# MECLabTUDA/Lifelong-nnUNet

Hardware: AMD Instinct MI355X
Metric: 3D patches/sec (whole node) + mean Dice vs ref, 5-level 3D Generic_UNet training step (higher is better)
Workload: dtype f16 (fp32 accumulate, fp32 master weights); 1 GPU; BASELINE configs[1]: nnUNetTrainerSequential.run_iteration, 160x192x160 patches, batch 2/GPU, num_pool 5, base 32, 3 logits; global_batch=2, parallelism=dp1, distinct_resident_batches=2, deterministic_wgrad=False

## Files before the change

lifelong-nnunet_amd/csrc/igemm_wgrad.hip:

```cpp
#include "lnn_common.h"
#include "igemm_gen.h"
#include <cstdlib>

namespace {

struct WTapTable {
    int ntaps;
    unsigned short pos_off[27];
    unsigned char slot[27];
};

struct WgradParams {
    const half_t* p;
    const half_t* q;
    const half_t* q2 = nullptr;
    int csplit = 0x7fffffff;
    float* dwp;
    int ld_p, ld_q;
    int N, Ld, Lh, Lw, Qd, Qh, Qw;
    int M, C, Mpad, Cpad;
    int tiles_z, tiles_y, tiles_x, tiles_total, tiles_per_block;
    int pad_lo;
    float* parts = nullptr;
    long parts_elems = 0, part_stride = 0;
// ... 748 lines not shown
                const char* qa = smem + 2 * ch * QX * 64 + tapaddr[ti];
                bq[buf][0] = lds_tr16(qa);
                bq[buf][1] = lds_tr16(qa + 256);
            }
        };
        rdA(0, 0);
        rdB(0, 0);
#pragma unroll
        for (int g = 0; g < NG; ++g) {
            const int ch = g / TPW, ti = g % TPW;
            if (g + 1 < NG) {
                rdB(g + 1, (g + 1) & 1);
                if ((g + 1) % TPW == 0) rdA((g + 1) / TPW, ((g + 1) / TPW) & 1);
            }
            if (wave + 8 * ti < NTAP) {
                const half4 b0 = bq[g & 1][0], b1 = bq[g & 1][1];
                const half8 b = {b0[0], b0[1], b0[2], b0[3], b1[0], b1[1], b1[2], b1[3]};
#pragma unroll
                for (int mp = 0; mp < MP; ++mp) acc[ti][mp] = __builtin_amdgcn_mfma_f32_32x32x16_f16(a[ch & 1][mp], b, acc[ti][mp], 0, 0, 0);
            }
#pragma unroll
            for (int e = 0; e < DPP; ++e) {
                const int d = g * DPP + e;
                if (d < nq) dma_q(nxt, rel0 + d / KPW, wrap(nbase + rel0 + d / KPW), d % KPW);
                else if (d == nq) dma_p(nxt, img ^ 1);
            }
            __builtin_amdgcn_sched_barrier(0);
        }
        wg_wait_all();
        __syncthreads();
        base = nbase;
        img ^= 1;
        cur = nxt;
    }
    const int c = c0 + (lane & 31);
#pragma unroll
    for (int ti = 0; ti < TPW; ++ti) {
        const int tap = wave + 8 * ti;
        if (tap < NTAP) {
            const long pbase_ = (long)tap * p.Mpad * p.Cpad;
#pragma unroll
            for (int mp = 0; mp < MP; ++mp) {
                if (m0 + mp * 32 >= p.Mpad) continue;
#pragma unroll
                for (int r = 0; r < 16; ++r) {
                    const int m = m0 + mp * 32 + 8 * (r >> 2) + 4 * hk + (r & 3);
                    wg_out(p, blk.chunk, 0, pbase_ + (long)m * p.Cpad + c, acc[ti][mp][r]);
                }
            }
        }
    }
}

int launch_wgrad_s1_v5(hipStream_t s, WgradParams& p) {
    constexpr int TZ = 4, TY = 8, TX = 8;
    p.tiles_z = lnn_cdiv(p.Ld, TZ); p.tiles_y = lnn_cdiv(p.Lh, TY); p.tiles_x = lnn_cdiv(p.Lw, TX);
    p.tiles_total = p.N * p.tiles_z * p.tiles_y * p.tiles_x;
    const int panels = (p.Mpad / 32) * (p.Cpad / 32);
    static int num_cu = 0;
    if (!num_cu) {
        int dev = 0;
        hipDeviceProp_t prop;
        num_cu = (hipGetDevice(&dev) == hipSuccess && hipGetDeviceProperties(&prop, dev) == hipSuccess) ? prop.multiProcessorCount : 256;
        hipFuncSetAttribute(reinterpret_cast<const void*>(igemm_wgrad_s1_v5_kernel), hipFuncAttributeMaxDynamicSharedMemorySize, 160 * 1024);
    }
    static int dbg4 = -1;
    static unsigned long long* dbgbuf4 = nullptr;
    if (dbg4 < 0) {
        const char* e = getenv("LNN_WGRAD_DEBUG"); dbg4 = e ? atoi(e) : 0;
        const char* b = getenv("LNN_WGRAD_PHASEBUF"); if ((dbg4 & 4) && b) dbgbuf4 = (unsigned long long*)strtoull(b, nullptr, 0);
    }
    p.debug = dbg4; p.dbgbuf = dbgbuf4;
    int tpb = lnn_cdiv((long)p.tiles_total * panels, lnn_cu_budget(num_cu));
    if (tpb < 1) tpb = 1;
    if (tpb > p.tiles_total) tpb = p.tiles_total;
    p.tiles_per_block = tpb;
    const unsigned chunks = (unsigned)lnn_cdiv(p.tiles_total, tpb);
    const dim3 grid = wg_grid(p, chunks, (unsigned)panels);
    const long slot_elems = 27L * p.Mpad * p.Cpad;
    if (int e = wg_prepare_parts(p, chunks, 2, slot_elems, "lnn_conv3d_wgrad(s1)")) return e;
    hipLaunchKernelGGL(igemm_wgrad_s1_v5_kernel, grid, dim3(512), (size_t)(12 * 7 * 1024 + 2 * 2 * 512 * 16), s, p);
    LNN_CHECK_LAUNCH("lnn_conv3d_wgrad(s1,v5)");
    return wg_reduce_parts(s, p, chunks, slot_elems, "lnn_conv3d_wgrad(s1,v5,reduce)");
}

template <int EXT>
int launch_wgrad_s2_v2(hipStream_t s, WgradParams& p, const char* name) {
    constexpr int TY = 8, TX = 8;
    constexpr int QZ = 1 + (EXT == 3), QY = TY + (EXT == 3), QX = TX + (EXT == 3);
    p.tiles_z = p.Ld; p.tiles_y = lnn_cdiv(p.Lh, TY); p.tiles_x = lnn_cdiv(p.Lw, TX);
    p.tiles_total = p.N * p.tiles_z * p.tiles_y * p.tiles_x;
    const int panels = lnn_cdiv(p.Mpad, 64) * (p.Cpad / 32);
    int tpb = lnn_cdiv((long)p.tiles_total * panels, 512);
    if (tpb < 1) tpb = 1;
    if (tpb > p.tiles_total) tpb = p.tiles_total;
    p.tiles_per_block = tpb;
    const size_t lds = (size_t)8 * QZ * QY * QX * 64 + (size_t)2 * 64 * 64;
    auto kern = igemm_wgrad_s2_v2_kernel<EXT>;
    static bool attr_set = false;
    if (!attr_set) {
        (void)hipFuncSetAttribute(reinterpret_cast<const void*>(kern), hipFuncAttributeMaxDynamicSharedMemorySize, 159 * 1024);
        attr_set = true;
    }
    const unsigned chunks = (unsigned)lnn_cdiv(p.tiles_total, tpb);
    const dim3 grid = wg_grid(p, chunks, (unsigned)panels);
    const long slot_elems = (long)(EXT * EXT * EXT) * p.Mpad * p.Cpad;
    if (int e = wg_prepare_parts(p, chunks, 1, slot_elems, name)) return e;
    hipLaunchKernelGGL(kern, grid, dim3(512), lds, s, p);
    LNN_CHECK_LAUNCH(name);
    return wg_reduce_parts(s, p, chunks, slot_elems, name);
}

template <int EXT>
int launch_wgrad_s2(hipStream_t s, WgradParams& p, const char* name) {
    static int s2s = -1;
    if (s2s < 0) { const char* e = getenv("LNN_WGRAD_S2S"); s2s = (e && e[0] == '0') ? 0 : 1; }
    constexpr int TY = 8, TX = 8, PY = 2 * (TY - 1) + EXT;
    const bool dma_ok = (long)PY * p.Qw * p.ld_q * 2 < 0x7fffffffL && (long)TY * p.Lw * p.ld_p * 2 < 0x7fffffffL;
    const bool one_panel_ext2 = EXT == 2 && lnn_cdiv(p.Mpad, 64) * (p.Cpad / 32) < 2;
    if (!s2s || !dma_ok || one_panel_ext2) return launch_wgrad_s2_v2<EXT>(s, p, name);
    constexpr int QY = TY + (EXT == 3), QX = TX + (EXT == 3), NPI = (4 * QY * QX * 64 + 1023) / 1024;
    p.tiles_z = p.Ld; p.tiles_y = lnn_cdiv(p.Lh, TY); p.tiles_x = lnn_cdiv(p.Lw, TX);
    p.tiles_total = p.N * p.tiles_z * p.tiles_y * p.tiles_x;
    const int panels = lnn_cdiv(p.Mpad, 64) * (p.Cpad / 32);
    static int num_cu = 0;
    if (!num_cu) {
        int dev = 0;
        hipDeviceProp_t prop;
        num_cu = (hipGetDevice(&dev) == hipSuccess && hipGetDeviceProperties(&prop, dev) == hipSuccess) ? prop.multiProcessorCount : 256;
    }
    int tpb = lnn_cdiv((long)p.tiles_total * panels, lnn_cu_budget(num_cu));
    if (tpb < 1) tpb = 1;
    if (tpb > p.tiles_total) tpb = p.tiles_total;
    p.tiles_per_block = tpb;
    const size_t lds = (size_t)2 * EXT * NPI * 1024 + (size_t)2 * 2 * 64 * 64;
    auto kern = igemm_wgrad_s2s_kernel<EXT>;
    static bool attr_set = false;
    if (!attr_set) {
        (void)hipFuncSetAttribute(reinterpret_cast<const void*>(kern), hipFuncAttributeMaxDynamicSharedMemorySize, 160 * 1024);
        attr_set = true;
    }
    const unsigned chunks = (unsigned)lnn_cdiv(p.tiles_total, tpb);
    const dim3 grid = wg_grid(p, chunks, (unsigned)panels);
    const long slot_elems = (long)(EXT * EXT * EXT) * p.Mpad * p.Cpad;
    if (int e = wg_prepare_parts(p, chunks, 1, slot_elems, name)) return e;
    hipLaunchKernelGGL(kern, grid, dim3(512), lds, s, p);
    LNN_CHECK_LAUNCH(name);
    return wg_reduce_parts(s, p, chunks, slot_elems, name);
}

int check_act_w(const void* ptr, int ld, int C, const char* what) {
    LNN_REQUIRE(ptr != nullptr, "%s: null pointer", what);
    LNN_REQUIRE(lnn_aligned16(ptr), "%s: pointer not 16-byte aligned", what);
    LNN_REQUIRE(C > 0 && C % 8 == 0, "%s: channel count %d must be a positive multiple of 8", what, C);
    LNN_REQUIRE(ld >= C && ld % 8 == 0, "%s: ld %d must be >= C (%d) and a multiple of 8", what, ld, C);
    return LNN_OK;
}

}

namespace {
__global__ void tr16_probe_kernel(float* out) {
    __shared__ __attribute__((aligned(16))) half_t img[256];
    for (int i = threadIdx.x; i < 256; i += 64) img[i] = (half_t)(float)i;
    __syncthreads();
    const half4 r = lds_tr16(reinterpret_cast<const char*>(img) + threadIdx.x * 8);
    for (int j = 0; j < 4; ++j) out[threadIdx.x * 4 + j] = (float)r[j];
}
}

extern "C" int lnn_debug_tr16_probe(lnn_stream_t s_, float* out256) {
    LNN_REQUIRE(out256 != nullptr, "lnn_debug_tr16_probe: null pointer");
    hipLaunchKernelGGL(tr16_probe_kernel, dim3(1), dim3(64), 0, (hipStream_t)s_, out256);
    LNN_CHECK_LAUNCH("lnn_debug_tr16_probe");
    return LNN_OK;
}

extern "C" size_t lnn_wgrad_panel_elems(int ntaps, int M, int KC) {
    return (size_t)ntaps * lnn_round_up(M, 32) * lnn_round_up(KC, 32);
}

namespace {
struct C1Fused {
    const void* gz; int ld_gz; const float *mean, *rstd, *gamma, *beta; float slope; const double* sums;
};
int conv3d_wgrad_impl(lnn_stream_t s_, const void* x, const void* x2, int c_a, int ld_x, const void* dy, int ld_dy, float* dwp, int N,
                      int Di, int Hi, int Wi, int C, int K, int stride, float* parts = nullptr, long parts_elems = 0,
                      const C1Fused* fused = nullptr) {
    hipStream_t s = (hipStream_t)s_;
    LNN_REQUIRE(stride == 1 || stride == 2, "lnn_conv3d_wgrad: stride %d unsupported", stride);
    LNN_REQUIRE(dwp != nullptr, "lnn_conv3d_wgrad: null panel");
    if (int e = check_act_w(dy, ld_dy, K, "lnn_conv3d_wgrad(dy)")) return e;
    WgradParams p{};
    p.p = (const half_t*)dy; p.q = (const half_t*)x; p.dwp = dwp; p.ld_p = ld_dy; p.ld_q = ld_x;
    p.parts = parts; p.parts_elems = parts_elems;
    if (x2) { p.q2 = (const half_t*)x2; p.csplit = c_a; }
    p.N = N; p.Qd = Di; p.Qh = Hi; p.Qw = Wi;
    p.Ld = (Di - 1) / stride + 1; p.Lh = (Hi - 1) / stride + 1; p.Lw = (Wi - 1) / stride + 1;
    p.M = K; p.C = C; p.Mpad = lnn_round_up(K, 32); p.Cpad = lnn_round_up(C, 32); p.pad_lo = 1;
    if (fused) {
        LNN_REQUIRE(C == 1, "lnn_conv3d_wgrad_c1_in_bwd: first layer (C == 1) only");
        p.gz = (const half_t*)fused->gz; p.ld_gz = fused->ld_gz; p.in_mean = fused->mean; p.in_rstd = fused->rstd;
        p.in_gamma = fused->gamma; p.in_beta = fused->beta; p.in_slope = fused->slope; p.in_sums = fused->sums;
    }
    if (C == 1) {
        LNN_REQUIRE(stride == 1 && x != nullptr, "lnn_conv3d_wgrad: C == 1 path needs stride 1");
        constexpr int TZ = 4, TY = 8;
        p.Cpad = 32;
        p.tiles_z = lnn_cdiv(p.Ld, TZ); p.tiles_y = lnn_cdiv(p.Lh, TY); p.tiles_x = lnn_cdiv(p.Lw, 8);
        p.tiles_total = N * p.tiles_z * p.tiles_y * p.tiles_x;
        int tpb = lnn_cdiv(p.tiles_total, 2048);
        if (tpb < 1) tpb = 1;
        p.tiles_per_block = tpb;
        dim3 grid((unsigned)lnn_cdiv(p.tiles_total, tpb), (unsigned)(p.Mpad / 32));
        const long slot_elems = (long)p.Mpad * 32;
        if (int e = wg_prepare_parts(p, grid.x, 4, slot_elems, "lnn_conv3d_wgrad(C=1)")) return e;
        if (p.gz) hipLaunchKernelGGL((wgrad_c1_kernel<TZ, TY, true>), grid, dim3(256), 0, s, p);
        else hipLaunchKernelGGL((wgrad_c1_kernel<TZ, TY, false>), grid, dim3(256), 0, s, p);
        LNN_CHECK_LAUNCH("lnn_conv3d_wgrad(C=1)");
        return wg_reduce_parts(s, p, grid.x, slot_elems, "lnn_conv3d_wgrad(C=1,reduce)");
    }
    if (int e = check_act_w(x, ld_x, x2 ? c_a : C, "lnn_conv3d_wgrad(x)")) return e;
    if (!x2 && lnn_gen_prefers(LNN_GEN_OP_WGRAD, (long)N * p.Ld * p.Lh * p.Lw)) {
        const int k3[3] = {3, 3, 3}, st3[3] = {stride, stride, stride};
        return lnn_gen_conv3d_wgrad(s, x, ld_x, dy, ld_dy, dwp, N, Di, Hi, Wi, C, K, k3, st3, parts, parts_elems);
    }
    p.taps.ntaps = 27;
    if (stride == 1) {
        constexpr int PY = 10, PX = 10;
        for (int t = 0; t < 27; ++t) {
            p.taps.pos_off[t] = (unsigned short)(((t / 9) * PY + (t / 3) % 3) * PX + t % 3);
            p.taps.slot[t] = (unsigned char)t;
        }
        LNN_REQUIRE(6L * p.Qh * p.Qw * p.ld_q * 2 < 0x7fffffffL && 4L * p.Lh * p.Lw * p.ld_p * 2 < 0x7fffffffL,
                    "lnn_conv3d_wgrad: a z-plane of %ld bytes is beyond the 2 GB window of the tile descriptors", (long)p.Qh * p.Qw * p.ld_q * 2);
        return launch_wgrad_s1_v5(s, p);
    }
    return launch_wgrad_s2<3>(s, p, "lnn_conv3d_wgrad(s2)");
}
}

extern "C" int lnn_conv3d_wgrad(lnn_stream_t s, const void* x, int ld_x, const void* dy, int ld_dy, float* dwp, int N,
                                int Di, int Hi, int Wi, int C, int K, int stride) {
    return conv3d_wgrad_impl(s, x, nullptr, 0, ld_x, dy, ld_dy, dwp, N, Di, Hi, Wi, C, K, stride);
}

extern "C" int lnn_conv3d_wgrad_c1_in_bwd(lnn_stream_t s, const void* x, const void* y, const void* dz, int ld_dz, float* dwp, int N,
                                          int D, int H, int W, int K, const float* mean, const float* rstd, const float* gamma,
                                          const float* beta, float slope, const double* ws, float* parts, long parts_elems) {
    LNN_REQUIRE(y && dz && lnn_aligned16(y) && lnn_aligned16(dz) && ld_dz >= K && ld_dz % 8 == 0, "lnn_conv3d_wgrad_c1_in_bwd: bad y / dz / ld_dz");
    LNN_REQUIRE(mean && rstd && gamma && beta && ws, "lnn_conv3d_wgrad_c1_in_bwd: null parameter");
    LNN_REQUIRE(parts == nullptr || lnn_aligned16(parts), "lnn_conv3d_wgrad_c1_in_bwd: scratch misaligned");
    const C1Fused f{dz, ld_dz, mean, rstd, gamma, beta, slope, ws};
    return conv3d_wgrad_impl(s, x, nullptr, 0, 1, y, K, dwp, N, D, H, W, 1, K, 1, parts, parts_elems, &f);
}

extern "C" int lnn_conv3d_wgrad_cat(lnn_stream_t s, const void* x_a, const void* x_b, int ld_x, int c_a, const void* dy, int ld_dy,
                                    float* dwp, int N, int Di, int Hi, int Wi, int C, int K) {
    LNN_REQUIRE(x_b != nullptr && lnn_aligned16(x_b), "lnn_conv3d_wgrad_cat: second tensor null/misaligned");
    LNN_REQUIRE(c_a > 0 && c_a < C && c_a % 32 == 0 && (C - c_a) % 8 == 0, "lnn_conv3d_wgrad_cat: split %d of %d channels must be a multiple of 32", c_a, C);
    LNN_REQUIRE(ld_x >= c_a && ld_x >= C - c_a, "lnn_conv3d_wgrad_cat: ld_x %d smaller than a part (%d / %d)", ld_x, c_a, C - c_a);
    return conv3d_wgrad_impl(s, x_a, x_b, c_a, ld_x, dy, ld_dy, dwp, N, Di, Hi, Wi, C, K, 1);
}

namespace {
int convT3d_k2s2_wgrad_impl(lnn_stream_t s_, const void* x, int ld_x, const void* dy, int ld_dy, float* dwp, int N, int D, int H, int W,
                            int C, int K, float* parts, long parts_elems);
}
extern "C" int lnn_convT3d_k2s2_wgrad(lnn_stream_t s, const void* x, int ld_x, const void* dy, int ld_dy, float* dwp,
                                      int N, int D, int H, int W, int C, int K) {
    return convT3d_k2s2_wgrad_impl(s, x, ld_x, dy, ld_dy, dwp, N, D, H, W, C, K, nullptr, 0);
}
extern "C" int lnn_conv3d_wgrad_det(lnn_stream_t s, const void* x, int ld_x, const void* dy, int ld_dy, float* dwp, int N, int Di, int Hi,
                                    int Wi, int C, int K, int stride, float* parts, long parts_elems) {
    LNN_REQUIRE(parts != nullptr && lnn_aligned16(parts), "lnn_conv3d_wgrad_det: scratch null/misaligned");
    return conv3d_wgrad_impl(s, x, nullptr, 0, ld_x, dy, ld_dy, dwp, N, Di, Hi, Wi, C, K, stride, parts, parts_elems);
}
extern "C" int lnn_conv3d_wgrad_cat_det(lnn_stream_t s, const void* x_a, const void* x_b, int ld_x, int c_a, const void* dy, int ld_dy,
                                        float* dwp, int N, int Di, int Hi, int Wi, int C, int K, float* parts, long parts_elems) {
    LNN_REQUIRE(parts != nullptr && lnn_aligned16(parts), "lnn_conv3d_wgrad_cat_det: scratch null/misaligned");
    LNN_REQUIRE(x_b != nullptr && lnn_aligned16(x_b), "lnn_conv3d_wgrad_cat_det: second tensor null/misaligned");
    LNN_REQUIRE(c_a > 0 && c_a < C && c_a % 32 == 0 && (C - c_a) % 8 == 0, "lnn_conv3d_wgrad_cat_det: split %d of %d channels must be a multiple of 32", c_a, C);
    LNN_REQUIRE(ld_x >= c_a && ld_x >= C - c_a, "lnn_conv3d_wgrad_cat_det: ld_x %d smaller than a part (%d / %d)", ld_x, c_a, C - c_a);
    return conv3d_wgrad_impl(s, x_a, x_b, c_a, ld_x, dy, ld_dy, dwp, N, Di, Hi, Wi, C, K, 1, parts, parts_elems);
}
extern "C" int lnn_convT3d_k2s2_wgrad_det(lnn_stream_t s, const void* x, int ld_x, const void* dy, int ld_dy, float* dwp, int N, int D,
                                          int H, int W, int C, int K, float* parts, long parts_elems) {
    LNN_REQUIRE(parts != nullptr && lnn_aligned16(parts), "lnn_convT3d_k2s2_wgrad_det: scratch null/misaligned");
    return convT3d_k2s2_wgrad_impl(s, x, ld_x, dy, ld_dy, dwp, N, D, H, W, C, K, parts, parts_elems);
}
namespace {
int convT3d_k2s2_wgrad_impl(lnn_stream_t s_, const void* x, int ld_x, const void* dy, int ld_dy, float* dwp, int N, int D, int H, int W,
                            int C, int K, float* parts, long parts_elems) {
    hipStream_t s = (hipStream_t)s_;
    LNN_REQUIRE(dwp != nullptr, "lnn_convT3d_k2s2_wgrad: null panel");
    if (int e = check_act_w(x, ld_x, C, "lnn_convT3d_k2s2_wgrad(x)")) return e;
    if (int e = check_act_w(dy, ld_dy, K, "lnn_convT3d_k2s2_wgrad(dy)")) return e;
    if (lnn_gen_prefers(LNN_GEN_OP_WGRAD, (long)N * D * H * W)) {
        const int st3[3] = {2, 2, 2};
        return lnn_gen_convT3d_wgrad(s, x, ld_x, dy, ld_dy, dwp, N, D, H, W, C, K, st3, parts, parts_elems);
    }
    WgradParams p{};
    p.p = (const half_t*)x; p.q = (const half_t*)dy; p.dwp = dwp; p.ld_p = ld_x; p.ld_q = ld_dy;
    p.parts = parts; p.parts_elems = parts_elems;
    p.N = N; p.Ld = D; p.Lh = H; p.Lw = W; p.Qd = 2 * D; p.Qh = 2 * H; p.Qw = 2 * W;
    p.M = C; p.C = K; p.Mpad = lnn_round_up(C, 32); p.Cpad = lnn_round_up(K, 32); p.pad_lo = 0;
    return launch_wgrad_s2<2>(s, p, "lnn_convT3d_k2s2_wgrad");
}
}
```

lifelong-nnunet_amd/csrc/lnn_debug.h:

```cpp
#ifndef LNN_DEBUG_H
#define LNN_DEBUG_H
#include "../../include/lnn_hip.h"
#ifdef __cplusplus
extern "C" {
#endif

int lnn_debug_tr16_probe(lnn_stream_t s, float* out256);

int lnn_debug_set_phase_buffer(void* dev_ptr_6x_u64);
int lnn_debug_force_conv_kernel(int which);
int lnn_debug_force_down2_kernel(int which);
int lnn_debug_set_v9_zseg(int segments);

int lnn_debug_set_k133_v9(int mode);
int lnn_debug_last_k133_on_v9(void);

int lnn_debug_set_gen_mode(int mode);

int lnn_debug_last_dgrad_reduce_fused(void);

int lnn_debug_set_cu_budget(int cus);

#ifdef __cplusplus
}
#endif
#endif
```

lifelong-nnunet_amd/native.py:

```python
from __future__ import annotations

import ctypes as C
import os

_HERE = os.path.dirname(os.path.abspath(__file__))
LIB_PATH = os.environ.get("LNN_LIB_PATH") or os.path.join(_HERE, "csrc", "liblnn_hip.so")

_p = C.c_void_p
_i = C.c_int
_l = C.c_long
_f = C.c_float
_sz = C.c_size_t

SIGNATURES = {
    "lnn_last_error": (C.c_char_p, []),
    "lnn_version": (_i, []),
    "lnn_device_info": (_i, [C.POINTER(_i), C.POINTER(_i), C.c_char_p, _i]),
    "lnn_pack_weights": (_i, [_p, _p, _p, _i, _i, _i, _l, _l, _l]),
    "lnn_packed_weight_elems": (_sz, [_i, _i, _i]),
    "lnn_conv3d_fwd": (_i, [_p, _p, _i, _p, _p, _p, _i, _i, _i, _i, _i, _i, _i, _i]),
    "lnn_conv3d_dgrad": (_i, [_p, _p, _i, _p, _p, _i, _i, _i, _i, _i, _i, _i, _i, _i]),
    "lnn_conv3d_wgrad": (_i, [_p, _p, _i, _p, _i, _p, _i, _i, _i, _i, _i, _i, _i]),
    "lnn_conv3d_fwd_cat": (_i, [_p, _p, _p, _i, _i, _p, _p, _p, _i, _i, _i, _i, _i, _i, _i]),
    "lnn_conv3d_fwd_in_stats": (_i, [_p, _p, _p, _i, _i, _p, _p, _p, _i, _i, _i, _i, _i, _i, _i, _f, _p, _p, _p, _p, _l]),
# ... 30 lines not shown
    "lnn_seg1x1_bwd_ws_floats": (_sz, [_i, _i]),
    "lnn_dice_ce_fwd": (_i, [_p, _p, _p, _i, _i, _l, _i, _f, _p, _p]),
    "lnn_dice_ce_fwd_ds": (_i, [_p, _p, _p, _i, _i, _l, _i, _f, _p, _p, _f, _p, _i]),
    "lnn_dice_ce_bwd": (_i, [_p, _p, _p, _i, _i, _l, _i, _f, _p, _f, _p, _f, _p]),
    "lnn_dice_ce_loss_from_totals": (_i, [_p, _p, _i, _i, _l, _i, _f, _p]),
    "lnn_dice_ce_ws_doubles": (_sz, [_i, _i]),
    "lnn_online_dice_counts": (_i, [_p, _p, _p, _i, _i, _l, _p]),
    "lnn_kl_logits": (_i, [_p, _p, _p, _i, _i, _l, _f, _p, _p]),
    "lnn_kl_logits_ws_doubles": (_sz, [_i]),
    "lnn_plop_pseudo_labels": (_i, [_p, _p, _p, _p, _f, _i, _i, _i, _i, _i, _p, _p, _p, _p]),
    "lnn_local_pod": (_i, [_p, _p, _p, _i, _i, _i, _i, _i, _l, _l, _l, _l, _l, _i, _f, _i, _p, _p, _p]),
    "lnn_ewc_penalty_fwd": (_i, [_p, _p, _p, _p, _l, _f, _p, _p]),
    "lnn_ewc_penalty_bwd": (_i, [_p, _p, _p, _p, _l, _f, _f, _p, _p]),
    "lnn_fisher_square": (_i, [_p, _p, _p, _l, _f]),
    "lnn_fisher_accumulate": (_i, [_p, _p, _p, _l, _f, _f]),
    "lnn_fisher_ema": (_i, [_p, _p, _p, _l, _f, _f]),
    "lnn_rw_update": (_i, [_p, _p, _p, _p, _p, _p, _l, _f, _f, _p, _f, _f, _i]),
    "lnn_target_ce_fwd": (_i, [_p, _p, _p, _i, _i, _i, _l, _f, _i, _f, _p, _p]),
    "lnn_target_ce_bwd": (_i, [_p, _p, _p, _i, _i, _i, _l, _f, _i, _f, _p, _f, _p, _p]),
    "lnn_softmax_accumulate": (_i, [_p, _p, _p, _p, _p] + [_i] * 11 + [_f, _i]),
    "lnn_softmax_finalize": (_i, [_p, _p, _p, _i, _l, _p]),
    "lnn_gradnorm_sumsq": (_i, [_p, _p, _l, _f, _p, _i]),
    "lnn_flat_reduce_ws_doubles": (_sz, []),
    "lnn_sgd_nesterov_step_clipped": (_i, [_p, _p, _p, _p, _l, _f, _f, _f, _f, _f, _p]),
    "lnn_sgd_nesterov_step": (_i, [_p, _p, _p, _p, _l, _f, _f, _f, _f, _i]),
    "lnn_cast_f32_to_h": (_i, [_p, _p, _p, _l]),
    "lnn_f32_conv3d_fwd": (_i, [_p, _p, _i, _p, _p, _p, _i, _i, _i, _i, _i, _i, _i, _i]),
    "lnn_f32_conv3d_dgrad": (_i, [_p, _p, _i, _p, _p, _i, _i, _i, _i, _i, _i, _i, _i, _i]),
    "lnn_f32_conv3d_wgrad": (_i, [_p, _p, _i, _p, _i, _p, _i, _i, _i, _i, _i, _i, _i]),
    "lnn_f32_convT3d_k2s2_fwd": (_i, [_p, _p, _i, _p, _p, _i, _i, _i, _i, _i, _i, _i]),
    "lnn_f32_convT3d_k2s2_dgrad": (_i, [_p, _p, _i, _p, _p, _i, _i, _i, _i, _i, _i, _i, _i]),
    "lnn_f32_convT3d_k2s2_wgrad": (_i, [_p, _p, _i, _p, _i, _p, _i, _i, _i, _i, _i, _i]),
    "lnn_f32_conv3d_fwd_g": (_i, [_p, _p, _i, _p, _p, _p, _i] + [_i] * 12),
    "lnn_f32_conv3d_dgrad_g": (_i, [_p, _p, _i, _p, _p, _i] + [_i] * 13),
    "lnn_f32_conv3d_wgrad_g": (_i, [_p, _p, _i, _p, _i, _p] + [_i] * 12),
    "lnn_f32_convT3d_fwd_g": (_i, [_p, _p, _i, _p, _p, _i] + [_i] * 9),
    "lnn_f32_convT3d_dgrad_g": (_i, [_p, _p, _i, _p, _p, _i] + [_i] * 10),
    "lnn_f32_convT3d_wgrad_g": (_i, [_p, _p, _i, _p, _i, _p] + [_i] * 9),
    "lnn_image_to_cl_h": (_i, [_p, _p, _p, _i, _i, _l, _i]),
    "lnn_f32_image_to_cl": (_i, [_p, _p, _p, _i, _i, _l, _i]),
    "lnn_f32_instnorm_lrelu_fwd": (_i, [_p, _p, _i, _p, _i, _i, _l, _i, _f, _p, _p, _p, _p, _f]),
    "lnn_f32_instnorm_lrelu_bwd": (_i, [_p, _p, _i, _p, _i, _i, _l, _i, _p, _p, _p, _p, _f, _p, _p, _p]),
    "lnn_f32_seg1x1_fwd": (_i, [_p, _p, _i, _p, _p, _i, _l, _i, _i]),
    "lnn_f32_seg1x1_bwd": (_i, [_p, _p, _i, _p, _p, _p, _i, _p, _i, _l, _i, _i, _i]),
    "lnn_debug_tr16_probe": (_i, [_p, _p]),
    "lnn_debug_set_phase_buffer": (_i, [_p]),
    "lnn_debug_force_conv_kernel": (_i, [_i]),
    "lnn_debug_force_down2_kernel": (_i, [_i]),
    "lnn_debug_set_v9_zseg": (_i, [_i]),
    "lnn_debug_set_k133_v9": (_i, [_i]),
    "lnn_debug_last_k133_on_v9": (_i, []),
    "lnn_debug_set_gen_mode": (_i, [_i]),
    "lnn_debug_last_dgrad_reduce_fused": (_i, []),
    "lnn_debug_set_cu_budget": (_i, [_i]),
    "lnn_conv3d_fwd_g": (_i, [_p, _p, _i, _p, _p, _p, _i] + [_i] * 12 + [_p, _l]),
    "lnn_conv3d_dgrad_g": (_i, [_p, _p, _i, _p, _p, _i] + [_i] * 13 + [_p, _l]),
    "lnn_conv3d_wgrad_g": (_i, [_p, _p, _i, _p, _i, _p] + [_i] * 12 + [_p, _l]),
    "lnn_convT3d_fwd_g": (_i, [_p, _p, _i, _p, _p, _i] + [_i] * 9 + [_p, _l]),
    "lnn_convT3d_dgrad_g": (_i, [_p, _p, _i, _p, _p, _i] + [_i] * 10 + [_p, _l]),
    "lnn_convT3d_wgrad_g": (_i, [_p, _p, _i, _p, _i, _p] + [_i] * 9 + [_p, _l]),
    "lnn_convT3d_k2s2_fwd_ws": (_i, [_p, _p, _i, _p, _p, _i, _i, _i, _i, _i, _i, _i, _p, _l]),
    "lnn_convT3d_k2s2_dgrad_ws": (_i, [_p, _p, _i, _p, _p, _i, _i, _i, _i, _i, _i, _i, _i, _p, _l]),
}

_lib = None


class NativeLibraryMissing(RuntimeError):
    pass


def lib():
    global _lib
    if _lib is None:
        if not os.path.exists(LIB_PATH):
            raise NativeLibraryMissing(
                f"{LIB_PATH} not found: build it with `python -c 'import __graft_entry__ as g; g.build()'` "
                f"(make -C lifelong-nnunet_amd/csrc).  There is no CPU / PyTorch fallback.")
        h = C.CDLL(LIB_PATH)
        for name, (res, args) in SIGNATURES.items():
            fn = getattr(h, name)
            fn.restype = res
            fn.argtypes = args
        _lib = h
    return _lib


def _ptr(t):
    if t is None:
        return None
    return t.data_ptr() if hasattr(t, "data_ptr") else int(t)


def stream_handle():
    import torch
    return torch.cuda.current_stream().cuda_stream


_fn_cache = {}


def call(name, *args):
    fn = _fn_cache.get(name)
    if fn is None:
        fn = _fn_cache[name] = getattr(lib(), name)
    conv = []
# ... 31 lines not shown
```

Before: 104.4 patches/s.

## Add whole-row band wgrad kernel for small deep-level stride-1 convolutions

Adds a new stride-1 weight-gradient kernel that tiles over two z-planes and a band of full-width y-rows sized to fit LDS. It double-buffers the activation halo and gradient tiles with async DMA interleaved into the MFMA loop, and picks a chunk count from a simple cost model that weighs parallelism against partial-sum reduction. It is selected by default for layers with at least 128 channels and small spatial extent (the deep UNet levels), where the existing 4x8x8 tiling wastes work on padding and has too few tiles. It adds more dispatch heuristics and debug hooks, and relies on the cost model choosing sensible chunking.

```diff
diff --git a/lifelong-nnunet_amd/csrc/igemm_wgrad.hip b/lifelong-nnunet_amd/csrc/igemm_wgrad.hip
--- a/lifelong-nnunet_amd/csrc/igemm_wgrad.hip
+++ b/lifelong-nnunet_amd/csrc/igemm_wgrad.hip
@@ -824,6 +824,167 @@
     }
 }
 
+struct WgMtGeo {
+    int TY, PY, PX, P;
+    int BV, TV, nch;
+    int zb, yb;
+    int nq, nd;
+    unsigned mpx, mpy, mw;
+};
+__global__ __launch_bounds__(512, 2) void igemm_wgrad_mt_kernel(const WgradParams p, const WgMtGeo g) {
+    constexpr int MP = 2, NTAP = 27, TPW = 4;
+    constexpr int OOB = (int)0x80000000;
+    extern __shared__ __attribute__((aligned(16))) char smem[];
+    const unsigned lds0 = (unsigned)(unsigned long long)(__attribute__((address_space(3))) char*)smem;
+    const int hb = g.nq * 1024, pb = g.nd * 1024;
+
+    const int tid = threadIdx.x, lane = tid & 63;
+    const int wave = __builtin_amdgcn_readfirstlane(tid >> 6);
+    const WgBlock blk = wg_block(p);
+    const int cpanels = p.Cpad / 32;
+    const int m0 = (blk.panel / cpanels) * 32 * MP, c0 = (blk.panel % cpanels) * 32;
+    const half_t* const qsrc = c0 >= p.csplit ? p.q2 : p.q;
+    const int cq = c0 >= p.csplit ? c0 - p.csplit : c0;
+    const int hk = lane >> 5, cb = 16 * ((lane >> 4) & 1), sj = (lane & 15) >> 2, sq = lane & 3;
+    const int chb = (cb + 4 * sq) * 2;
+    const int p_addr = (8 * hk + sj) * 64 + chb;
+
+    floatx16 acc[TPW][MP];
+#pragma unroll
+    for (int i = 0; i < TPW; ++i)
+#pragma unroll
+        for (int a = 0; a < MP; ++a)
+#pragma unroll
+            for (int j = 0; j < 16; ++j) acc[i][a][j] = 0.f;
+
+    const int t_begin = blk.chunk * p.tiles_per_block;
+    const int t_end = min(t_begin + p.tiles_per_block, p.tiles_total);
+    if (t_begin >= t_end) return;
+
+    const int tyw = g.TY * p.Lw;
+    int* const vrow = reinterpret_cast<int*>(smem + 2 * hb + 2 * pb);
+    for (int v = tid; v < g.TV; v += 512) {
+        const int z = v >= tyw ? 1 : 0, r = v - z * tyw;
+        const int y = (int)(((unsigned)r * g.mw) >> 20), x = r - y * p.Lw;
+        vrow[v] = v < g.BV ? ((z * g.PY + y) * g.PX + x) * 64 : 0;
+    }
+
+    const long qsample = (long)p.Qd * p.Qh * p.Qw * p.ld_q, psample = (long)p.Ld * p.Lh * p.Lw * p.ld_p;
+    struct Tile { int n, z0, y0; };
+    auto decode = [&](int tile) {
+        const int ybi = tile % g.yb, r = tile / g.yb;
+        return Tile{r / g.zb, 2 * (r % g.zb), ybi * g.TY};
+    };
+    auto dma = [&](const Tile& t, int j, int img) {
+        const int c8 = lane & 3;
+        if (j < g.nq) {
+            const int pos = (j * 64 + lane) >> 2;
+            const int row = (int)(((unsigned)pos * g.mpx) >> 20), px = pos - row * g.PX;
+            const int pz = (int)(((unsigned)row * g.mpy) >> 20), py = row - pz * g.PY;
+            const int iz = t.z0 - 1 + pz, iy = t.y0 - 1 + py, ix = px - 1;
+            const bool ok = pos < g.P && (unsigned)iz < (unsigned)p.Qd && (unsigned)iy < (unsigned)p.Qh && (unsigned)ix < (unsigned)p.Qw &&
+                            c0 + c8 * 8 < p.C;
+            const int off = ok ? (((iz * p.Qh + iy) * p.Qw + ix) * p.ld_q + c8 * 8) * 2 : OOB;
+            wg_dma16(wg_rsrc_n(qsrc + t.n * qsample + cq, 0x7fffffffu), __builtin_amdgcn_readfirstlane(lds0 + img * hb + j * 1024), off);
+        } else if (j < g.nq + g.nd) {
+            const int jj = j - g.nq, vv = (jj * 64 + lane) >> 2;
+            const int mp = vv >= g.TV ? 1 : 0, v = vv - mp * g.TV;
+            const int z = v >= tyw ? 1 : 0, r = v - z * tyw;
+            const int y = (int)(((unsigned)r * g.mw) >> 20);
+            const bool ok = v < g.BV && t.z0 + z < p.Ld && t.y0 + y < p.Lh && m0 + mp * 32 + c8 * 8 < p.M;
+            const int off = ok ? ((((t.z0 + z) * p.Lh + t.y0) * p.Lw + r) * p.ld_p + mp * 32 + c8 * 8) * 2 : OOB;
+            wg_dma16(wg_rsrc_n(p.p + t.n * psample + m0, 0x7fffffffu), __builtin_amdgcn_readfirstlane(lds0 + 2 * hb + img * pb + jj * 1024), off);
+        }
+    };
+    const int ni = (g.nq + g.nd + 7) >> 3;
+    const int dpc = (ni + g.nch - 1) / g.nch;
+
+    int tapoff[TPW];
+#pragma unroll
+    for (int ti = 0; ti < TPW; ++ti) {
+        const int tap = min(wave + 8 * ti, NTAP - 1);
+        tapoff[ti] = (((tap / 9) * g.PY + (tap / 3) % 3) * g.PX + tap % 3) * 64 + chb;
+    }
+
+    Tile cur = decode(t_begin);
+    for (int i = 0; i < ni; ++i) dma(cur, 8 * i + wave, 0);
+    wg_wait_all();
+    __syncthreads();
+
+    int img = 0;
+#pragma unroll 1
+    for (int tile = t_begin; tile < t_end; ++tile) {
+        const bool more = tile + 1 < t_end;
+        const Tile nxt = more ? decode(tile + 1) : cur;
+        const char* const hl = smem + img * hb;
+        const char* const pl = smem + 2 * hb + img * pb + p_addr;
+        const int* const vr = vrow + 8 * hk + sj;
+        int di = more ? 0 : ni;
+        half8 a[2][MP], b[2][TPW];
+        auto rd = [&](int ch, int buf, int r0, int r1) {
+#pragma unroll
+            for (int mp = 0; mp < MP; ++mp) {
+                const half4 a0 = lds_tr16(pl + mp * g.TV * 64 + ch * 1024), a1 = lds_tr16(pl + mp * g.TV * 64 + ch * 1024 + 256);
+                a[buf][mp] = half8{a0[0], a0[1], a0[2], a0[3], a1[0], a1[1], a1[2], a1[3]};
+            }
+#pragma unroll
+            for (int ti = 0; ti < TPW; ++ti) {
+                if (ti < 3 || wave < NTAP - 24) {
+                    const half4 b0 = lds_tr16(hl + r0 + tapoff[ti]), b1 = lds_tr16(hl + r1 + tapoff[ti]);
+                    b[buf][ti] = half8{b0[0], b0[1], b0[2], b0[3], b1[0], b1[1], b1[2], b1[3]};
+                }
+            }
+        };
+        rd(0, 0, vr[0], vr[4]);
+        const int c1 = min(1, g.nch - 1);
+        int r0 = vr[16 * c1], r1 = vr[16 * c1 + 4];
+#pragma unroll 1
+        for (int ch2 = 0; ch2 < g.nch; ch2 += 2) {
+#pragma unroll
+            for (int h = 0; h < 2; ++h) {
+                const int ch = ch2 + h;
+                if (ch < g.nch) {
+                    const int chn = min(ch + 1, g.nch - 1), chnn = min(ch + 2, g.nch - 1);
+                    rd(chn, h ^ 1, r0, r1);
+                    r0 = vr[16 * chnn]; r1 = vr[16 * chnn + 4];
+                    __builtin_amdgcn_sched_barrier(0);
+#pragma unroll
+                    for (int ti = 0; ti < TPW; ++ti) {
+                        if (ti < 3 || wave < NTAP - 24) {
+#pragma unroll
+                            for (int mp = 0; mp < MP; ++mp)
+                                acc[ti][mp] = __builtin_amdgcn_mfma_f32_32x32x16_f16(a[h][mp], b[h][ti], acc[ti][mp], 0, 0, 0);
+                        }
+                    }
+                    __builtin_amdgcn_sched_barrier(0);
+                    for (int e = 0; e < dpc && di < ni; ++e, ++di) dma(nxt, 8 * di + wave, img ^ 1);
+                }
+            }
+        }
+        wg_wait_all();
+        __syncthreads();
+        img ^= 1;
+        cur = nxt;
+    }
+    const int c = c0 + (lane & 31);
+#pragma unroll
+    for (int ti = 0; ti < TPW; ++ti) {
+        const int tap = wave + 8 * ti;
+        if (tap < NTAP) {
+            const long pbase_ = (long)tap * p.Mpad * p.Cpad;
+#pragma unroll
+            for (int mp = 0; mp < MP; ++mp) {
+                if (m0 + mp * 32 >= p.Mpad) continue;
+#pragma unroll
+                for (int r = 0; r < 16; ++r) {
+                    const int m = m0 + mp * 32 + 8 * (r >> 2) + 4 * hk + (r & 3);
+                    wg_out(p, blk.chunk, 0, pbase_ + (long)m * p.Cpad + c, acc[ti][mp][r]);
+                }
+            }
+        }
+    }
+}
+
 int launch_wgrad_s1_v5(hipStream_t s, WgradParams& p) {
     constexpr int TZ = 4, TY = 8, TX = 8;
     p.tiles_z = lnn_cdiv(p.Ld, TZ); p.tiles_y = lnn_cdiv(p.Lh, TY); p.tiles_x = lnn_cdiv(p.Lw, TX);
@@ -921,6 +1082,83 @@
     return wg_reduce_parts(s, p, chunks, slot_elems, name);
 }
 
+constexpr int WG_MT_LDS = 160 * 1024;
+constexpr long WG_MT_SCRATCH = 64L * 1024 * 1024;
+bool wgrad_mt_geometry(const WgradParams& p, WgMtGeo& g) {
+    if (p.Lw > 256 || p.Lh < 1) return false;
+    long best = -1;
+    for (int ty = p.Lh; ty >= 1; --ty) {
+        const int bv = 2 * ty * p.Lw, tv = lnn_round_up(bv, 16), P = 4 * (ty + 2) * (p.Lw + 2);
+        const int nq = lnn_cdiv(P, 16), nd = tv / 8;
+        if (2L * (nq + nd) * 1024 + 4L * tv > WG_MT_LDS) continue;
+        const long cost = (long)lnn_cdiv(p.Lh, ty) * tv;
+        if (best >= 0 && cost >= best) continue;
+        best = cost;
+        g.TY = ty; g.PY = ty + 2; g.PX = p.Lw + 2; g.P = P; g.BV = bv; g.TV = tv; g.nch = tv / 16; g.nq = nq; g.nd = nd;
+    }
+    if (best < 0) return false;
+    g.zb = lnn_cdiv(p.Ld, 2); g.yb = lnn_cdiv(p.Lh, g.TY);
+    g.mpx = (1u << 20) / g.PX + 1; g.mpy = (1u << 20) / g.PY + 1; g.mw = (1u << 20) / p.Lw + 1;
+    return true;
+}
+bool wgrad_mt_supported(const WgradParams& p) {
+    WgMtGeo g;
+    if (p.Ld != p.Qd || p.Lh != p.Qh || p.Lw != p.Qw || p.pad_lo != 1 || p.gz) return false;
+    if ((double)p.Qd * p.Qh * p.Qw * p.ld_q * 2.0 >= 2147483648.0 || (double)p.Ld * p.Lh * p.Lw * p.ld_p * 2.0 >= 2147483648.0) return false;
+    return wgrad_mt_geometry(p, g);
+}
+
+int g_force_wgrad = -1, g_last_wgrad = 0;
+bool use_wgrad_mt(const WgradParams& p) {
+    if (!wgrad_mt_supported(p)) return false;
+    if (g_force_wgrad >= 0) return g_force_wgrad == 10;
+    static int v = -2;
+    if (v == -2) {
+        const char* e = getenv("LNN_WGRAD_MT");
+        v = e ? (e[0] == '1' ? 1 : 0) : -1;
+    }
+    if (v == 0) return false;
+    if (v == 1) return true;
+    return p.C >= 128 && p.M >= 128 && (long)p.Ld * p.Lh * p.Lw <= 10L * 12 * 10;
+}
+
+int launch_wgrad_mt(hipStream_t s, WgradParams& p) {
+    WgMtGeo g;
+    LNN_REQUIRE(wgrad_mt_geometry(p, g), "lnn_conv3d_wgrad(mt): no band of a %d x %d plane fits the LDS images", p.Lh, p.Lw);
+    p.tiles_z = g.zb; p.tiles_y = g.yb; p.tiles_x = 1;
+    p.tiles_total = p.N * g.zb * g.yb;
+    const int panels = lnn_cdiv(p.Mpad, 64) * (p.Cpad / 32);
+    const size_t lds = (size_t)2 * (g.nq + g.nd) * 1024 + (size_t)4 * g.TV;
+    static int num_cu = 0;
+    if (!num_cu) {
+        int dev = 0;
+        hipDeviceProp_t prop;
+        const hipError_t e = hipFuncSetAttribute(reinterpret_cast<const void*>(igemm_wgrad_mt_kernel),
+                                                 hipFuncAttributeMaxDynamicSharedMemorySize, WG_MT_LDS);
+        LNN_REQUIRE(e == hipSuccess, "lnn_conv3d_wgrad(mt): cannot reserve %d bytes of LDS: %s", WG_MT_LDS, hipGetErrorString(e));
+        num_cu = (hipGetDevice(&dev) == hipSuccess && hipGetDeviceProperties(&prop, dev) == hipSuccess) ? prop.multiProcessorCount : 256;
+    }
+    const long slot_elems = 27L * p.Mpad * p.Cpad;
+    const int max_chunks = WG_MT_SCRATCH / slot_elems > 1 ? (int)(WG_MT_SCRATCH / slot_elems) : 1;
+    static int cap = -1;
+    if (cap < 0) { const char* e = getenv("LNN_WGRAD_MT_CHUNKS"); cap = e && atoi(e) > 0 ? atoi(e) : 0; }
+    const int cus = lnn_cu_budget(num_cu);
+    int tpb = p.tiles_total;
+    double best = 0.0;
+    for (int c = 1; c <= p.tiles_total && c <= max_chunks && (!cap || c <= cap); ++c) {
+        const int t = lnn_cdiv(p.tiles_total, c), cc = lnn_cdiv(p.tiles_total, t);
+        const double cost = (double)lnn_cdiv((long)panels * cc, cus) * t * g.nch * 0.37 + cc * (slot_elems * 4e-6) * 1.0;
+        if (c == 1 || cost < best) { best = cost; tpb = t; }
+    }
+    p.tiles_per_block = tpb;
+    const unsigned chunks = (unsigned)lnn_cdiv(p.tiles_total, tpb);
+    const dim3 grid = wg_grid(p, chunks, (unsigned)panels);
+    if (int e = wg_prepare_parts(p, chunks, 1, slot_elems, "lnn_conv3d_wgrad(s1,mt)")) return e;
+    hipLaunchKernelGGL(igemm_wgrad_mt_kernel, grid, dim3(512), lds, s, p, g);
+    LNN_CHECK_LAUNCH("lnn_conv3d_wgrad(s1,mt)");
+    return wg_reduce_parts(s, p, chunks, slot_elems, "lnn_conv3d_wgrad(s1,mt,reduce)");
+}
+
 int check_act_w(const void* ptr, int ld, int C, const char* what) {
     LNN_REQUIRE(ptr != nullptr, "%s: null pointer", what);
     LNN_REQUIRE(lnn_aligned16(ptr), "%s: pointer not 16-byte aligned", what);
@@ -947,6 +1185,13 @@
     LNN_CHECK_LAUNCH("lnn_debug_tr16_probe");
     return LNN_OK;
 }
+
+extern "C" int lnn_debug_force_wgrad_kernel(int which) {
+    LNN_REQUIRE(which == -1 || which == 5 || which == 10, "lnn_debug_force_wgrad_kernel: %d is not one of -1, 5, 10", which);
+    g_force_wgrad = which;
+    return LNN_OK;
+}
+extern "C" int lnn_debug_last_wgrad_kernel(void) { return g_last_wgrad; }
 
 extern "C" size_t lnn_wgrad_panel_elems(int ntaps, int M, int KC) {
     return (size_t)ntaps * lnn_round_up(M, 32) * lnn_round_up(KC, 32);
@@ -1006,7 +1251,8 @@
         }
         LNN_REQUIRE(6L * p.Qh * p.Qw * p.ld_q * 2 < 0x7fffffffL && 4L * p.Lh * p.Lw * p.ld_p * 2 < 0x7fffffffL,
                     "lnn_conv3d_wgrad: a z-plane of %ld bytes is beyond the 2 GB window of the tile descriptors", (long)p.Qh * p.Qw * p.ld_q * 2);
-        return launch_wgrad_s1_v5(s, p);
+        g_last_wgrad = use_wgrad_mt(p) ? 10 : 5;
+        return g_last_wgrad == 10 ? launch_wgrad_mt(s, p) : launch_wgrad_s1_v5(s, p);
     }
     return launch_wgrad_s2<3>(s, p, "lnn_conv3d_wgrad(s2)");
 }
diff --git a/lifelong-nnunet_amd/csrc/lnn_debug.h b/lifelong-nnunet_amd/csrc/lnn_debug.h
--- a/lifelong-nnunet_amd/csrc/lnn_debug.h
+++ b/lifelong-nnunet_amd/csrc/lnn_debug.h
@@ -19,6 +19,9 @@
 
 int lnn_debug_last_dgrad_reduce_fused(void);
 
+int lnn_debug_force_wgrad_kernel(int which);
+int lnn_debug_last_wgrad_kernel(void);
+
 int lnn_debug_set_cu_budget(int cus);
 
 #ifdef __cplusplus
diff --git a/lifelong-nnunet_amd/native.py b/lifelong-nnunet_amd/native.py
--- a/lifelong-nnunet_amd/native.py
+++ b/lifelong-nnunet_amd/native.py
@@ -106,6 +106,8 @@
     "lnn_debug_last_k133_on_v9": (_i, []),
     "lnn_debug_set_gen_mode": (_i, [_i]),
     "lnn_debug_last_dgrad_reduce_fused": (_i, []),
+    "lnn_debug_force_wgrad_kernel": (_i, [_i]),
+    "lnn_debug_last_wgrad_kernel": (_i, []),
     "lnn_debug_set_cu_budget": (_i, [_i]),
     "lnn_conv3d_fwd_g": (_i, [_p, _p, _i, _p, _p, _p, _i] + [_i] * 12 + [_p, _l]),
     "lnn_conv3d_dgrad_g": (_i, [_p, _p, _i, _p, _p, _i] + [_i] * 13 + [_p, _l]),
```

After: 105.2 patches/s (median of 6 runs). Within noise of the previous version (+0.8%).

## Add small-spatial wgrad kernel that splits by weight panel and z-tap group

Applied to the files above, without the earlier changes.

Adds a dedicated weight-gradient kernel for deep, small-spatial layers (few voxels, many channel panels). It assigns each block a (panel, z-tap group) work item, keeps the whole XY plane of both operands in LDS with double-buffered DMA stages, and accumulates all 9 (or 4) in-plane taps in registers. Results are reduced across waves through LDS and added directly into the weight panel, so no partials buffer or separate reduce launch is needed. In exchange it has low parallelism when items are few, does a read-modify-write of dw, and is gated by voxel-count thresholds and an env switch.

```diff
diff --git a/lifelong-nnunet_amd/csrc/igemm_wgrad.hip b/lifelong-nnunet_amd/csrc/igemm_wgrad.hip
--- a/lifelong-nnunet_amd/csrc/igemm_wgrad.hip
+++ b/lifelong-nnunet_amd/csrc/igemm_wgrad.hip
@@ -824,6 +824,161 @@
     }
 }
 
+struct WgSmallPlan {
+    int nz;
+    int sh, sw;
+    int qslot;
+    int pbytes;
+    int stage_bytes;
+    int stages_per_sample, items, per_xcd, slots;
+    int c_major;
+    unsigned rcp_sw, rcp_lw, rcp_lhw;
+};
+__device__ __forceinline__ unsigned wg_udiv(unsigned x, unsigned rcp) { return rcp ? __umulhi(x, rcp) : x; }
+
+template <int S, int EXT>
+__global__ __launch_bounds__(512, 1) void igemm_wgrad_small_kernel(const WgradParams p, const WgSmallPlan sp) {
+    constexpr int NTG = EXT * EXT, TR = EXT == 3 ? 3 : 4;
+    constexpr int OOB = (int)0x80000000;
+    constexpr int KQ = 10;
+    extern __shared__ __attribute__((aligned(16))) char smem[];
+    const unsigned lds0 = (unsigned)(unsigned long long)(__attribute__((address_space(3))) char*)smem;
+
+    const int tid = threadIdx.x, lane = tid & 63;
+    const int wave = __builtin_amdgcn_readfirstlane(tid >> 6);
+    const int hk = lane >> 5, cb = 16 * ((lane >> 4) & 1), sj = (lane & 15) >> 2, sq = lane & 3;
+    const int chb = (cb + 4 * sq) * 2;
+    const int p_lane = (8 * hk + sj) * 64 + chb;
+    const int cpanels = p.Cpad / 32, mpanels = p.Mpad / 32;
+    const int lhw = p.Lh * p.Lw, qi = sp.qslot >> 10;
+    const long qplane = (long)p.Qh * p.Qw * p.ld_q;
+    const int xcd = blockIdx.x & 7, slot0 = blockIdx.x >> 3;
+    const int nstages = p.N * sp.stages_per_sample;
+    const int pv = ((lane >> 2) * p.ld_p + (lane & 3) * 8) * 2;
+    int qv[KQ];
+#pragma unroll
+    for (int k = 0; k < KQ; ++k) {
+        const int pos = (wave + 8 * k) * 16 + (lane >> 2);
+        const int sy = (int)wg_udiv((unsigned)pos, sp.rcp_sw), sx = pos - sy * sp.sw;
+        const int iy = sy - p.pad_lo, ix = sx - p.pad_lo;
+        const bool ok = sy < sp.sh && (unsigned)iy < (unsigned)p.Qh && (unsigned)ix < (unsigned)p.Qw;
+        qv[k] = ok ? ((iy * p.Qw + ix) * p.ld_q + (lane & 3) * 8) * 2 : OOB;
+    }
+
+#pragma unroll 1
+    for (int k = slot0; k < sp.per_xcd; k += sp.slots) {
+        const int item = xcd * sp.per_xcd + k;
+        if (item >= sp.items) break;
+        const int grp = item % EXT, panel = item / EXT;
+        const int m0 = (sp.c_major ? panel % mpanels : panel / cpanels) * 32, c0 = (sp.c_major ? panel / mpanels : panel % cpanels) * 32;
+        const half_t* const qsrc = c0 >= p.csplit ? p.q2 : p.q;
+        const int cq = c0 >= p.csplit ? c0 - p.csplit : c0;
+
+        floatx16 acc[NTG];
+#pragma unroll
+        for (int i = 0; i < NTG; ++i)
+#pragma unroll
+            for (int j = 0; j < 16; ++j) acc[i][j] = 0.f;
+
+        auto issue = [&](int st, int buf) {
+            const int n = st / sp.stages_per_sample, z0 = (st - n * sp.stages_per_sample) * sp.nz;
+            const int nzc = min(sp.nz, p.Ld - z0), nvox = nzc * lhw, kg = (nvox + 15) >> 4;
+            const unsigned base = lds0 + buf * sp.stage_bytes;
+            const half_t* const porg = p.p + ((long)n * p.Ld + z0) * lhw * p.ld_p + m0;
+            for (int j = wave; j < kg; j += 8)
+                wg_dma16(wg_rsrc_n(porg + (long)j * 16 * p.ld_p, (unsigned)(nvox - 16 * j) * p.ld_p * 2), base + j * 1024, pv);
+            for (int zi = 0; zi < nzc; ++zi) {
+                const int iz = S * (z0 + zi) + grp - p.pad_lo;
+                const bool zin = (unsigned)iz < (unsigned)p.Qd;
+                const uint4v rq = wg_rsrc_n(qsrc + ((long)n * p.Qd + (zin ? iz : 0)) * qplane + cq, zin ? 0x7fffffffu : 0u);
+#pragma unroll
+                for (int k = 0; k < KQ; ++k)
+                    if (wave + 8 * k < qi) wg_dma16(rq, base + sp.pbytes + zi * sp.qslot + (wave + 8 * k) * 1024, qv[k]);
+            }
+        };
+
+        issue(0, 0);
+        wg_wait_all();
+        __syncthreads();
+        int rot = 0;
+#pragma unroll 1
+        for (int st = 0; st < nstages; ++st) {
+            const int buf = st & 1;
+            if (st + 1 < nstages) issue(st + 1, buf ^ 1);
+            const int zs = st % sp.stages_per_sample;
+            const int nvox = min(sp.nz, p.Ld - zs * sp.nz) * lhw, kg = (nvox + 15) >> 4;
+            const char* const pl = smem + buf * sp.stage_bytes;
+            const char* const ql = pl + sp.pbytes;
+            auto rd = [&](int g, half8& a, half8 (&b)[NTG]) {
+                int qa[2];
+#pragma unroll
+                for (int h = 0; h < 2; ++h) {
+                    const int v = min(16 * g + 8 * hk + sj + 4 * h, nvox - 1);
+                    const int z = (int)wg_udiv((unsigned)v, sp.rcp_lhw), rem = v - z * lhw;
+                    const int y = (int)wg_udiv((unsigned)rem, sp.rcp_lw), x = rem - y * p.Lw;
+                    qa[h] = z * sp.qslot + (S * y * sp.sw + S * x) * 64 + chb;
+                }
+                const half4 a0 = lds_tr16(pl + g * 1024 + p_lane), a1 = lds_tr16(pl + g * 1024 + 256 + p_lane);
+                a = half8{a0[0], a0[1], a0[2], a0[3], a1[0], a1[1], a1[2], a1[3]};
+#pragma unroll
+                for (int t = 0; t < NTG; ++t) {
+                    const int off = ((t / EXT) * sp.sw + t % EXT) * 64;
+                    const half4 b0 = lds_tr16(ql + qa[0] + off), b1 = lds_tr16(ql + qa[1] + off);
+                    b[t] = half8{b0[0], b0[1], b0[2], b0[3], b1[0], b1[1], b1[2], b1[3]};
+                }
+            };
+            auto mm = [&](const half8& a, const half8 (&b)[NTG]) {
+#pragma unroll
+                for (int t = 0; t < NTG; ++t) acc[t] = __builtin_amdgcn_mfma_f32_32x32x16_f16(a, b[t], acc[t], 0, 0, 0);
+            };
+#pragma unroll 1
+            for (int g = (wave - rot) & 7; g < kg; g += 8) {
+                half8 a, b[NTG];
+                rd(g, a, b);
+                mm(a, b);
+            }
+            rot = (rot + kg) & 7;
+            wg_wait_all();
+            __syncthreads();
+        }
+
+        float* const epi = reinterpret_cast<float*>(smem);
+        constexpr int NR = (NTG + TR - 1) / TR, EPT = TR * 2;
+        auto out_idx = [&](int r0, int i) {
+            const int e = i * 512 + tid, tt = e >> 10, el = e & 1023, r = el >> 6, le = el & 63;
+            const int m = m0 + 8 * (r >> 2) + 4 * (le >> 5) + (r & 3), c = c0 + (le & 31);
+            return (long)(grp * NTG + r0 + tt) * p.Mpad * p.Cpad + (long)m * p.Cpad + c;
+        };
+        float old[NR][EPT];
+#pragma unroll
+        for (int rd_ = 0; rd_ < NR; ++rd_)
+#pragma unroll
+            for (int i = 0; i < EPT; ++i)
+                if (rd_ * TR + (i >> 1) < NTG) old[rd_][i] = p.dwp[out_idx(rd_ * TR, i)];
+#pragma unroll
+        for (int rd_ = 0; rd_ < NR; ++rd_) {
+            const int r0 = rd_ * TR;
+#pragma unroll
+            for (int tt = 0; tt < TR; ++tt)
+                if (r0 + tt < NTG)
+#pragma unroll
+                    for (int r = 0; r < 16; ++r) epi[((tt * 8 + wave) * 16 + r) * 64 + lane] = acc[r0 + tt][r];
+            __syncthreads();
+#pragma unroll
+            for (int i = 0; i < EPT; ++i) {
+                if (r0 + (i >> 1) < NTG) {
+                    const int e = i * 512 + tid, tt = e >> 10, el = e & 1023;
+                    float sum = epi[tt * 8 * 1024 + el];
+#pragma unroll
+                    for (int w = 1; w < 8; ++w) sum += epi[(tt * 8 + w) * 1024 + el];
+                    p.dwp[out_idx(r0, i)] = old[rd_][i] + sum;
+                }
+            }
+            __syncthreads();
+        }
+    }
+}
+
 int launch_wgrad_s1_v5(hipStream_t s, WgradParams& p) {
     constexpr int TZ = 4, TY = 8, TX = 8;
     p.tiles_z = lnn_cdiv(p.Ld, TZ); p.tiles_y = lnn_cdiv(p.Lh, TY); p.tiles_x = lnn_cdiv(p.Lw, TX);
@@ -921,6 +1076,68 @@
     return wg_reduce_parts(s, p, chunks, slot_elems, name);
 }
 
+int g_force_wgrad_small = -1;
+int g_last_wgrad_small = 0;
+
+unsigned wg_rcp(int d) { return d <= 1 ? 0u : (unsigned)((0x100000000ULL + (unsigned)d - 1) / (unsigned)d); }
+
+bool wgrad_small_plan(const WgradParams& p, int S, int EXT, int slots_budget, WgSmallPlan& sp) {
+    if (p.parts || p.gz || p.C == 1) return false;
+    if (p.M % 32 || p.C % 32 || p.ld_p % 8 || p.ld_q % 8 || !lnn_aligned16(p.p) || !lnn_aligned16(p.q)) return false;
+    if (p.q2 && (p.csplit % 32 || !lnn_aligned16(p.q2))) return false;
+    const long lhw = (long)p.Lh * p.Lw;
+    sp.sh = S * (p.Lh - 1) + EXT; sp.sw = S * (p.Lw - 1) + EXT;
+    const long qslot = ((long)sp.sh * sp.sw * 64 + 1023) / 1024 * 1024;
+    constexpr long HALF = 80 * 1024;
+    int nz = 0;
+    while (nz < p.Ld && ((nz + 1) * lhw * 64 + 1023) / 1024 * 1024 + (nz + 1) * qslot <= HALF) ++nz;
+    if (nz < 1 || qslot > 79 * 1024) return false;
+    if ((long)nz * lhw * p.ld_p * 2 >= 0x7fffffffL || (long)p.Qh * p.Qw * p.ld_q * 2 >= 0x7fffffffL) return false;
+    sp.nz = nz; sp.qslot = (int)qslot;
+    sp.pbytes = (int)((nz * lhw * 64 + 1023) / 1024 * 1024);
+    sp.stage_bytes = sp.pbytes + nz * sp.qslot;
+    sp.stages_per_sample = lnn_cdiv(p.Ld, nz);
+    sp.items = (p.Mpad / 32) * (p.Cpad / 32) * EXT;
+    sp.c_major = (long)p.Qd * p.Qh * p.Qw * p.C >= (long)p.Ld * lhw * p.M ? 1 : 0;
+    sp.per_xcd = lnn_cdiv(sp.items, 8);
+    sp.slots = slots_budget < 1 ? 1 : (slots_budget < sp.per_xcd ? slots_budget : sp.per_xcd);
+    sp.rcp_sw = wg_rcp(sp.sw); sp.rcp_lw = wg_rcp(p.Lw); sp.rcp_lhw = wg_rcp((int)lhw);
+    return true;
+}
+
+constexpr int WG_SMALL_MAX_VOXELS = 1600, WG_SMALL_MAX_VOXELS_T = 1200, WG_SMALL_MIN_ITEMS = 12;
+bool use_wgrad_small(const WgradParams& p, const WgSmallPlan& sp, int EXT) {
+    if (g_force_wgrad_small >= 0) return g_force_wgrad_small == 1;
+    static int off = -1;
+    if (off < 0) { const char* e = getenv("LNN_WGRAD_SMALL"); off = (e && e[0] == '0') ? 1 : 0; }
+    if (off) return false;
+    return (long)p.Ld * p.Lh * p.Lw <= (EXT == 3 ? WG_SMALL_MAX_VOXELS : WG_SMALL_MAX_VOXELS_T) && sp.items >= WG_SMALL_MIN_ITEMS;
+}
+
+template <int S, int EXT>
+int try_wgrad_small(hipStream_t s, WgradParams& p, const char* name) {
+    static int num_cu = 0;
+    static bool attr_ok = false;
+    auto kern = igemm_wgrad_small_kernel<S, EXT>;
+    if (!num_cu) {
+        int dev = 0;
+        hipDeviceProp_t prop;
+        num_cu = (hipGetDevice(&dev) == hipSuccess && hipGetDeviceProperties(&prop, dev) == hipSuccess) ? prop.multiProcessorCount : 256;
+        attr_ok = hipFuncSetAttribute(reinterpret_cast<const void*>(kern), hipFuncAttributeMaxDynamicSharedMemorySize, 160 * 1024) == hipSuccess;
+        (void)hipGetLastError();
+    }
+    if (!attr_ok) return 0;
+    WgSmallPlan sp{};
+    if (!wgrad_small_plan(p, S, EXT, lnn_cu_budget(num_cu) / 8, sp) || !use_wgrad_small(p, sp, EXT)) return 0;
+    constexpr int EPI = (EXT == 3 ? 3 : 4) * 8 * 4096;
+    const size_t lds = (size_t)(2 * sp.stage_bytes > EPI ? 2 * sp.stage_bytes : EPI);
+    hipLaunchKernelGGL(kern, dim3(8u * sp.slots), dim3(512), lds, s, p, sp);
+    hipError_t e = hipGetLastError();
+    if (e != hipSuccess) { lnn_set_error("%s(small): launch failed: %s", name, hipGetErrorString(e)); return LNN_ERR_LAUNCH; }
+    g_last_wgrad_small = 1;
+    return 1;
+}
+
 int check_act_w(const void* ptr, int ld, int C, const char* what) {
     LNN_REQUIRE(ptr != nullptr, "%s: null pointer", what);
     LNN_REQUIRE(lnn_aligned16(ptr), "%s: pointer not 16-byte aligned", what);
@@ -947,6 +1164,13 @@
     LNN_CHECK_LAUNCH("lnn_debug_tr16_probe");
     return LNN_OK;
 }
+
+extern "C" int lnn_debug_force_wgrad_small(int mode) {
+    LNN_REQUIRE(mode >= -1 && mode <= 1, "lnn_debug_force_wgrad_small: %d is not one of -1, 0, 1", mode);
+    g_force_wgrad_small = mode;
+    return LNN_OK;
+}
+extern "C" int lnn_debug_last_wgrad_small(void) { return g_last_wgrad_small; }
 
 extern "C" size_t lnn_wgrad_panel_elems(int ntaps, int M, int KC) {
     return (size_t)ntaps * lnn_round_up(M, 32) * lnn_round_up(KC, 32);
@@ -960,6 +1184,7 @@
                       int Di, int Hi, int Wi, int C, int K, int stride, float* parts = nullptr, long parts_elems = 0,
                       const C1Fused* fused = nullptr) {
     hipStream_t s = (hipStream_t)s_;
+    g_last_wgrad_small = 0;
     LNN_REQUIRE(stride == 1 || stride == 2, "lnn_conv3d_wgrad: stride %d unsupported", stride);
     LNN_REQUIRE(dwp != nullptr, "lnn_conv3d_wgrad: null panel");
     if (int e = check_act_w(dy, ld_dy, K, "lnn_conv3d_wgrad(dy)")) return e;
@@ -997,6 +1222,7 @@
         const int k3[3] = {3, 3, 3}, st3[3] = {stride, stride, stride};
         return lnn_gen_conv3d_wgrad(s, x, ld_x, dy, ld_dy, dwp, N, Di, Hi, Wi, C, K, k3, st3, parts, parts_elems);
     }
+    if (const int r = stride == 1 ? try_wgrad_small<1, 3>(s, p, "lnn_conv3d_wgrad") : try_wgrad_small<2, 3>(s, p, "lnn_conv3d_wgrad")) return r < 0 ? r : LNN_OK;
     p.taps.ntaps = 27;
     if (stride == 1) {
         constexpr int PY = 10, PX = 10;
@@ -1065,6 +1291,7 @@
 int convT3d_k2s2_wgrad_impl(lnn_stream_t s_, const void* x, int ld_x, const void* dy, int ld_dy, float* dwp, int N, int D, int H, int W,
                             int C, int K, float* parts, long parts_elems) {
     hipStream_t s = (hipStream_t)s_;
+    g_last_wgrad_small = 0;
     LNN_REQUIRE(dwp != nullptr, "lnn_convT3d_k2s2_wgrad: null panel");
     if (int e = check_act_w(x, ld_x, C, "lnn_convT3d_k2s2_wgrad(x)")) return e;
     if (int e = check_act_w(dy, ld_dy, K, "lnn_convT3d_k2s2_wgrad(dy)")) return e;
@@ -1077,6 +1304,7 @@
     p.parts = parts; p.parts_elems = parts_elems;
     p.N = N; p.Ld = D; p.Lh = H; p.Lw = W; p.Qd = 2 * D; p.Qh = 2 * H; p.Qw = 2 * W;
     p.M = C; p.C = K; p.Mpad = lnn_round_up(C, 32); p.Cpad = lnn_round_up(K, 32); p.pad_lo = 0;
+    if (const int r = try_wgrad_small<2, 2>(s, p, "lnn_convT3d_k2s2_wgrad")) return r < 0 ? r : LNN_OK;
     return launch_wgrad_s2<2>(s, p, "lnn_convT3d_k2s2_wgrad");
 }
 }
diff --git a/lifelong-nnunet_amd/csrc/lnn_debug.h b/lifelong-nnunet_amd/csrc/lnn_debug.h
--- a/lifelong-nnunet_amd/csrc/lnn_debug.h
+++ b/lifelong-nnunet_amd/csrc/lnn_debug.h
@@ -19,6 +19,9 @@
 
 int lnn_debug_last_dgrad_reduce_fused(void);
 
+int lnn_debug_force_wgrad_small(int mode);
+int lnn_debug_last_wgrad_small(void);
+
 int lnn_debug_set_cu_budget(int cus);
 
 #ifdef __cplusplus
diff --git a/lifelong-nnunet_amd/native.py b/lifelong-nnunet_amd/native.py
--- a/lifelong-nnunet_amd/native.py
+++ b/lifelong-nnunet_amd/native.py
@@ -106,6 +106,8 @@
     "lnn_debug_last_k133_on_v9": (_i, []),
     "lnn_debug_set_gen_mode": (_i, [_i]),
     "lnn_debug_last_dgrad_reduce_fused": (_i, []),
+    "lnn_debug_force_wgrad_small": (_i, [_i]),
+    "lnn_debug_last_wgrad_small": (_i, []),
     "lnn_debug_set_cu_budget": (_i, [_i]),
     "lnn_conv3d_fwd_g": (_i, [_p, _p, _i, _p, _p, _p, _i] + [_i] * 12 + [_p, _l]),
     "lnn_conv3d_dgrad_g": (_i, [_p, _p, _i, _p, _p, _i] + [_i] * 13 + [_p, _l]),
```

New measurement: 88.35 before, 88.28 after. No clear change (-0.1%).
